# apache/datafusion

Hardware: AMD Instinct MI355X
Metric: tpch_q3_hash_join_rows_per_sec (higher is better)
Workload: dtype int64 keys / decimal128 payload; 1 GPU; INNER hash-join orders⋈lineitem on o_orderkey, TPC-H SF100, Q3 payload (o_orderdate,o_shippriority,l_orderkey,l_extendedprice,l_discount), device-resident inputs; build_rows=150000000, probe_rows=599960064, output_rows=599960064, join_table=rank_map, probe=single_pass_unordered, parallelism=single GPU, exchange=none

## Files before the change

### datafusion_amd/csrc/internal.hpp

```cpp
#pragma once
#include <atomic>
#include <hip/hip_runtime.h>

#include <chrono>
#include <cstdint>
#include <cstring>
#include <map>
#include <memory>
#include <mutex>
#include <stdexcept>
#include <string>
#include <thread>
#include <vector>

#include "../../include/dfgpu.h"

namespace dfgpu {

struct Error : std::runtime_error {
  using std::runtime_error::runtime_error;
};

void set_last_error(const std::string& msg);

// ... 236 lines not shown
  thread_metrics().rows_out += t->nrows;
  return reinterpret_cast<dfgpu_table_t>(t);
}

Column alloc_column(const dfgpu_field& f, const std::string& name, int64_t n, bool with_validity = false);
inline Column alloc_like(const Column& src, int64_t n, bool with_validity = false) {
  Column c = alloc_column(src.field, src.name, n, with_validity);
  c.dict = src.dict;
  return c;
}

inline dfgpu_table_t wrap_quiet(Table* t) { return reinterpret_cast<dfgpu_table_t>(t); }

void scan_mask_popcounts(const uint64_t* mask, const uint64_t* valid, int64_t nrows, uint64_t* out_prefix);
void scan_u32(const uint32_t* in, int64_t n, uint64_t* out_prefix);
void scan_bitmap_words_tab(const uint64_t* words, int64_t n_words, uint64_t* out_prefix, void* out_tab);
uint64_t read_u64(const uint64_t* dev);

Table compact_table(const Table& in, const std::vector<int>& cols, const uint64_t* mask, const uint64_t* mask_valid);
Column gather_column(const Column& in, const int64_t* idx, int64_t n, bool idx_may_be_null);
std::vector<Column> gather_columns(const Table& in, const std::vector<int>& cols, const int64_t* idx, int64_t n, bool idx_may_be_null, const uint32_t* idx32 = nullptr);
struct PackLayout;
bool plan_record_layout(const Table& in, const std::vector<int>& cols, PackLayout& L, int& R, std::vector<int>& order);
Column bool_as_u8(const Column& c, int64_t n);
void and_bitmaps(const uint64_t* a, const uint64_t* b, int64_t nw, uint64_t* out);
void count_nulls(Column& c);

struct Datum {
  Column col;
  std::string str;
  bool scalar = false;
// ... 66 lines not shown
```

### datafusion_amd/csrc/join.hip

```cpp
#include <thread>
#include <functional>
#include <cstdlib>

#include "device.hpp"
#include "internal.hpp"
#include "grouped.hpp"

namespace dfgpu {

Table compact_table(const Table& in, const std::vector<int>& cols, const uint64_t* mask, const uint64_t* mask_valid);
void pack_bytes_to_bitmap(const uint8_t* bytes, int64_t n, uint64_t* words);

enum TableKind : int { KIND_HASH = 0, KIND_ARRAY = 1, KIND_RANK = 2, KIND_RADIX = 3, KIND_FLAT = 4, KIND_FLAT16 = 5,
                       KIND_RETURNED = 6 };
template <int KIND> constexpr bool kind_is_flat() { return KIND == KIND_FLAT || KIND == KIND_FLAT16; }
template <int KIND> constexpr bool kind_is_direct() { return KIND == KIND_ARRAY || KIND == KIND_RANK; }

struct FlatLayout {
  int n;
  uint8_t off[MAX_KEYS];
  uint8_t width[MAX_KEYS];
  int8_t null_bit[MAX_KEYS];
};
constexpr double RANK_MAP_MIN_KEY_DENSITY = 1.0 / 256.0;
// ... 38 lines not shown
  const uint64_t* rank_prefix;
  const uint32_t* rank_perm;
  uint64_t am_offset, am_size, hash_mask;
  int null_equals_null;
  int force_collisions;
  const uint64_t* row_mask;
  const uint4* flat;
  FlatLayout flat_layout;
  int flat_shift;
  uint64_t flat_mask;
  const uint32_t* ret_dest;
  const uint8_t* ret_rec;
  int ret_R;
};

constexpr int ROWPRED_MAX = 2;
struct RowPred {
  const void* data[ROWPRED_MAX];
  const uint64_t* valid[ROWPRED_MAX];
  long long lit[ROWPRED_MAX];
  uint8_t width[ROWPRED_MAX], is_unsigned[ROWPRED_MAX], op[ROWPRED_MAX];
  int n;
};
template <bool NT, int W>
__device__ __forceinline__ void rowpred_load_words(const RowPred& q, int i, int64_t w0, int64_t np, unsigned lane, long long (&v)[W]) {
  const int width = q.width[i];
  if (width == 8) {
    const long long* d = reinterpret_cast<const long long*>(q.data[i]);
#pragma unroll
    for (int j = 0; j < W; j++) {
// ... 184 lines not shown
      lo[j] = load_key<KT>(k, i < n ? i : n - 1);
    }
#pragma unroll
    for (int j = 0; j < BUILD_UNROLL; j++) {
      int64_t i = i0 + j * stride;
      ok[j] = i < n;
      if (HASV) ok[j] = ok[j] && bit_at(k.valid, i < n ? i : n - 1);
    }
#pragma unroll
    for (int j = 0; j < BUILD_UNROLL; j++) {
      if (!ok[j]) continue;
      const uint64_t idx = lo[j] - offset;
      const unsigned long long bit = 1ull << (idx & 63);
      (void)__hip_atomic_fetch_or(&bits[idx >> 6], bit, __ATOMIC_RELAXED, __HIP_MEMORY_SCOPE_AGENT);
    }
  }
}
template <int KT, bool HASV>
__global__ __launch_bounds__(BLOCK) void k_rank_setbytes(KeyCol k, int64_t n, uint64_t offset, uint8_t* __restrict__ bytes) {
  const int64_t stride = (int64_t)gridDim.x * BLOCK;
  for (int64_t i0 = (int64_t)blockIdx.x * BLOCK + threadIdx.x; i0 < n; i0 += stride * BUILD_UNROLL) {
    uint64_t lo[BUILD_UNROLL];
#pragma unroll
    for (int j = 0; j < BUILD_UNROLL; j++) {
      const int64_t i = i0 + j * stride;
      lo[j] = load_key<KT>(k, i < n ? i : n - 1);
    }
#pragma unroll
    for (int j = 0; j < BUILD_UNROLL; j++) {
      const int64_t i = i0 + j * stride;
// ... 20 lines not shown
    const uint64_t idx = gkeys[i] - offset;
    const unsigned long long bit = 1ull << (idx & 63);
    const unsigned long long old = atomicOr(&rb_words[(idx >> 6) - w0], bit);
    dup |= (old & bit) != 0;
  }
  if (dup) *dup_flag = 1;
  __syncthreads();
  for (int i = threadIdx.x; i < nw; i += RB_THREADS) {
    const unsigned long long w = rb_words[i];
    if (i == 0 || i == nw - 1) {
      if (w) atomicOr(&bits[w0 + i], w);
    } else {
      bits[w0 + i] = w;
    }
  }
}
__global__ __launch_bounds__(BLOCK) void k_rank_interleave(const uint64_t* __restrict__ bits, const uint64_t* __restrict__ prefix, int64_t n_words, ulonglong2* __restrict__ tab) {
  for (int64_t w = (int64_t)blockIdx.x * BLOCK + threadIdx.x; w < n_words; w += (int64_t)gridDim.x * BLOCK) tab[w] = make_ulonglong2(bits[w], prefix[w]);
}
__global__ __launch_bounds__(BLOCK) void k_rank_perm_tab(KeyCol k, int64_t n, uint64_t offset, const ulonglong2* __restrict__ tab, uint32_t* __restrict__ perm) {
  for (int64_t i = (int64_t)blockIdx.x * BLOCK + threadIdx.x; i < n; i += (int64_t)gridDim.x * BLOCK) {
    if (k.valid && !bit_at(k.valid, i)) continue;
    uint64_t lo, hi;
    load_words(k, i, lo, hi);
    const uint64_t idx = lo - offset;
    const ulonglong2 e = tab[idx >> 6];
    perm[(uint32_t)e.y + (uint32_t)__popcll(e.x & ((1ull << (idx & 63)) - 1ull))] = (uint32_t)i;
  }
}

// ... 355 lines not shown
    ok[j] = p < np;
    idx[j] = (keys_in ? keys_in[j] : load_key<KT, NT>(k, ok[j] ? p : np - 1)) - c.am_offset;
    if (pre) ok[j] = ok[j] && pre[j];
    else if (c.row_mask) ok[j] = ok[j] && ((c.row_mask[w0 + j] >> lane) & 1ull);
  }
  if (k.valid) {
    uint64_t vw[N];
#pragma unroll
    for (int j = 0; j < N; j++) {
      const int64_t p = ((w0 + j) << 6) + lane;
      vw[j] = k.valid[(p < np ? p : np - 1) >> 6];
    }
#pragma unroll
    for (int j = 0; j < N; j++) ok[j] = ok[j] && ((vw[j] >> lane) & 1ull);
  }
  const uint64_t* tab = c.rank_bits;
  uint64_t bits[N];
#pragma unroll
  for (int j = 0; j < N; j++) {
    ok[j] = ok[j] && idx[j] < c.am_size;
    bits[j] = tab[ok[j] ? (idx[j] >> 6) : 0];
  }
#pragma unroll
  for (int j = 0; j < N; j++) word[j] = ballot64(ok[j] && ((bits[j] >> (idx[j] & 63)) & 1ull));
}

__device__ __forceinline__ uint32_t out_count(int join_type, uint32_t nmatch) {
  switch (join_type) {
    case DFGPU_JOIN_INNER: case DFGPU_JOIN_LEFT: return nmatch;
    case DFGPU_JOIN_RIGHT: case DFGPU_JOIN_FULL: return nmatch ? nmatch : 1u;
    case DFGPU_JOIN_RIGHT_SEMI: return nmatch ? 1u : 0u;
    case DFGPU_JOIN_RIGHT_ANTI: return nmatch ? 0u : 1u;
    case DFGPU_JOIN_RIGHT_MARK: return 1u;
    default: return 0u;
  }
}
// ... 573 lines not shown
  __syncthreads();
  const uint32_t round_rows = agg - base < (uint32_t)EL_CAP ? agg - base : (uint32_t)EL_CAP;
  for (uint32_t q0 = threadIdx.x; q0 < round_rows; q0 += BLOCK) {
    const uint32_t q = base + q0;
    const int64_t prow = (w_base << 6) + s_row[q0];
    int64_t brow = 0;
    uint64_t key = 0;
    if (cols.n_build > 0 || cols.key_col >= 0) {
      key = load_key<KT>(k, prow);
      if (cols.n_build > 0) {
        const uint64_t idx = key - c.am_offset;
        if (KIND == KIND_ARRAY) {
          brow = (int64_t)c.heads[idx] - 1;
        } else {
          uint64_t bw, pre;
          if (c.rank_tab) {
            const ulonglong2 e = c.rank_tab[idx >> 6];
            bw = e.x;
            pre = e.y;
          } else {
            bw = c.rank_bits[idx >> 6];
            pre = c.rank_prefix[idx >> 6];
          }
          const uint32_t rank = (uint32_t)pre + (uint32_t)__popcll(bw & ((1ull << (idx & 63)) - 1ull));
          brow = c.rank_perm ? (int64_t)c.rank_perm[rank] : (int64_t)rank;
        }
      }
    }
    const int64_t d = (int64_t)(out0 + q);
#pragma unroll
    for (int c0 = 0; c0 < MAX_JOIN_COLS; c0 += 4) {
      if (c0 >= cols.n) continue;
      uint4 v[4];
#pragma unroll
      for (int u = 0; u < 4; u++) {
        if (c0 + u >= cols.n) continue;
        int ci = c0 + u + cols.n_build;
        if (ci >= cols.n) ci -= cols.n;
// ... 339 lines not shown
  }
  if (kind == KIND_RETURNED) {
    f(std::integral_constant<int, KIND_RETURNED>{}, std::integral_constant<int, KT_ANY>{});
    return;
  }
  with_key_type(probe_key_type, [&](auto kt) {
    if (kind == KIND_ARRAY) f(std::integral_constant<int, KIND_ARRAY>{}, kt);
    else f(std::integral_constant<int, KIND_RANK>{}, kt);
  });
}

static void ensure_rank_tab(JoinTable& jt) {
  if (jt.kind != KIND_RANK) return;
  std::lock_guard<std::mutex> lk(jt.tab_mu);
  if (jt.rank_tab) return;
  Runtime& r = rt();
  const int64_t n_words = (int64_t)((jt.am_size - 1) >> 6) + 1;
  BufPtr tab = make_buf((size_t)n_words * 16);
  {
    ProfileScope ps("join_build_rank_interleave", n_words * 16);
    k_rank_interleave<<<grid_for(n_words, BLOCK), BLOCK, 0, r.stream>>>(jt.rank_bits->as<uint64_t>(), jt.rank_prefix->as<uint64_t>(), n_words, tab->as<ulonglong2>());
    DFGPU_HIP(hipGetLastError());
  }
  call_epilogue();
  jt.rank_tab = tab;
  std::lock_guard<std::mutex> lk2(jt.mu);
  jt.info.table_bytes += n_words * 16;
}

static void ensure_rank_perm(JoinTable& jt) {
  if (jt.kind != KIND_RANK || !jt.rank_needs_perm) return;
  ensure_rank_tab(jt);
  std::lock_guard<std::mutex> lk(jt.mu);
  if (jt.rank_perm) return;
  Runtime& r = rt();
  const int64_t nb = jt.build.nrows;
  const KeySet ks = make_keyset(jt.build, jt.key_cols);
  BufPtr perm = make_buf((size_t)std::max<int64_t>(nb, 1) * 4);
  {
    ProfileScope ps("join_build_rank_perm", nb * (ks.c[0].width + 4));
    k_rank_perm_tab<<<grid_for(nb, BLOCK), BLOCK, 0, r.stream>>>(ks.c[0], nb, jt.am_offset, jt.rank_tab->as<ulonglong2>(), perm->as<uint32_t>());
    DFGPU_HIP(hipGetLastError());
// ... 4 lines not shown
}

static ProbeCtx make_ctx(JoinTable& jt, const Table& probe, const std::vector<int>& pk, bool need_build_rows = true, bool want_tab = true) {
  if (want_tab) ensure_rank_tab(jt);
  if (need_build_rows) ensure_rank_perm(jt);
  ProbeCtx c{};
  c.bkeys = make_keyset(jt.build, jt.key_cols);
  c.pkeys = make_keyset(probe, pk);
  for (int i = 0; i < c.bkeys.n; i++) {
    int bt = c.bkeys.c[i].type == DFGPU_DATE32 ? DFGPU_INT32 : c.bkeys.c[i].type;
    int pt = c.pkeys.c[i].type == DFGPU_DATE32 ? DFGPU_INT32 : c.pkeys.c[i].type;
    DFGPU_CHECK(bt == pt, "join key types differ between build and probe side (the planner inserts casts)");
  }
  c.heads = jt.heads ? jt.heads->as<uint32_t>() : nullptr;
  c.next = jt.next ? jt.next->as<uint32_t>() : nullptr;
  c.rank_tab = jt.rank_tab ? jt.rank_tab->as<ulonglong2>() : nullptr;
  c.rank_bits = jt.rank_bits ? jt.rank_bits->as<uint64_t>() : nullptr;
  c.rank_prefix = jt.rank_prefix ? jt.rank_prefix->as<uint64_t>() : nullptr;
  c.rank_perm = need_build_rows && jt.rank_perm ? jt.rank_perm->as<uint32_t>() : nullptr;
  c.am_offset = jt.am_offset;
  c.am_size = jt.am_size;
  c.hash_mask = jt.hash_mask;
  c.flat = jt.flat ? jt.flat->as<uint4>() : nullptr;
  c.flat_layout = jt.flat_layout;
  c.flat_shift = jt.flat_shift;
  c.flat_mask = jt.flat_mask;
  c.null_equals_null = jt.null_equality == DFGPU_NULL_EQUALS_NULL;
  c.force_collisions = jt.force_collisions;
  return c;
}

static Column mark_column(const uint8_t* bytes, int64_t n) {
  dfgpu_field f{};
// ... 154 lines not shown
        std::atomic_store(&const_cast<Column&>(kc).stats, std::make_shared<ColStats>(ColStats{res.smin, res.smax, (int64_t)res.valid, res.unsorted == 0, res.descends == 0}));
      }
    }
  }
  const double dense = have_stats ? (double)nb / ((double)range + 1.0) : 0.0;
  bool am_ok = have_stats && !(range >= (uint64_t)opts.perfect_hash_join_small_build_threshold && dense <= opts.perfect_hash_join_min_key_density);
  if (opts.table_mode == 2) am_ok = have_stats;
  am_ok = am_ok && range < (1ull << 34);
  bool rank_ok = have_stats && (opts.table_mode == 0 || opts.table_mode == 3) && range < (1ull << 40) &&
                 (range < (uint64_t)opts.perfect_hash_join_small_build_threshold || dense >= RANK_MAP_MIN_KEY_DENSITY || opts.table_mode == 3);
  DFGPU_CHECK(!speculated || rank_ok, "internal: speculative build statistics outside the rank map's gate");
  DFGPU_CHECK(!(opts.table_mode == 2 && !am_ok), "direct-address join table requested but not applicable");
  DFGPU_CHECK(!(opts.table_mode == 3 && !rank_ok), "rank-map join table requested but not applicable");
  constexpr int64_t MALL_BYTES = (int64_t)256 << 20;

  BufPtr flag = make_zero_buf(4);
  int dup = 0;
  bool flat_wide = false;
  if (rank_ok && !ascending && !speculated && opts.table_mode == 0 && opts.probe_mode == 4 && ks.n == 1 && nb * 8 > MALL_BYTES && nb >= ((int64_t)1 << 22)) {
    const int64_t m = (int64_t)1 << 18;
    const uint64_t slots = (uint64_t)1 << 20;
    BufPtr table = make_zero_buf((size_t)slots * 8);
    {
      ProfileScope ps("join_build_sample_duplicates", m * 2 * ks.c[0].width);
      with_key_type(ks.c[0].type, [&](auto kt) {
        k_sample_duplicates<decltype(kt)::value><<<grid_for(2 * m, BLOCK), BLOCK, 0, r.stream>>>(ks.c[0], nb, nb / m, m, table->as<unsigned long long>(), slots - 1, flag->as<int>());
      });
      DFGPU_HIP(hipGetLastError());
    }
    int seen = 0;
    d2h(&seen, flag->ptr, 4);
    if (seen) {
      dup = 1;
      rank_ok = false;
      DFGPU_HIP(hipMemsetAsync(flag->ptr, 0, 4, r.stream));
    }
  }
  if (rank_ok) {
    const int64_t n_words = (int64_t)(range >> 6) + 1;
    jt->rank_bits = make_zero_buf((size_t)n_words * 8);
    {
      ProfileScope ps("join_build_rank_map", nb * ks.c[0].width);
      int g = std::min(grid_for(nb, BLOCK * BUILD_UNROLL), 2048);
      unsigned long long* bits = jt->rank_bits->as<unsigned long long>();
      KeyCol kc0 = ks.c[0];
      BufPtr grouped_keys;
      constexpr int RB_BITS = 10;
      const bool lds_bits = !ascending && nb > (1 << 22) && n_words * 8 > ((int64_t)16 << 20) && (range >> RB_BITS) < (1ull << 20) - 64;
      if (lds_bits) {
        const GroupSpec gs = group_spec((uint64_t)kmin, range + 1, 1 << RB_BITS);
        GroupedRows gr = group_rows_by_key(kc0, nb, gs, RB_BITS, nullptr, true, false, {}, {}, "join_build_group_keys");
        const int P = 1 << RB_BITS;
        std::vector<uint64_t> gfirst((size_t)P + 1);
        uint64_t max_span = 0;
        for (int q = 0; q <= P; q++) {
          const unsigned __int128 v = ((((unsigned __int128)(unsigned)q) << 64) + gs.mul - 1) / gs.mul;
          gfirst[(size_t)q] = v > (unsigned __int128)(range + 1) || q == P ? range + 1 : (uint64_t)v;
          if (q) max_span = std::max(max_span, gfirst[(size_t)q] - gfirst[(size_t)q - 1]);
        }
        BufPtr d_first = make_buf(gfirst.size() * 8);
        h2d_async(d_first->ptr, gfirst.data(), gfirst.size() * 8);
        const size_t lds = (size_t)((max_span >> 6) + 2) * 8;
        DFGPU_HIP(hipFuncSetAttribute(reinterpret_cast<const void*>(k_rank_bits_grouped), hipFuncAttributeMaxDynamicSharedMemorySize, (int)lds));
        k_rank_bits_grouped<<<P, RB_THREADS, lds, r.stream>>>(gr.keys->as<uint64_t>(), gr.bounds->as<uint64_t>(), d_first->as<uint64_t>(), (uint64_t)kmin, bits, flag->as<int>());
        DFGPU_HIP(hipGetLastError());
        DFGPU_HIP(hipStreamSynchronize(r.stream));
      } else {
      if (!ascending && !kc0.valid && kc0.width == 8 && nb > (1 << 22) && n_words * 8 > ((int64_t)16 << 20)) {
        const Column& kcol = build.cols[(size_t)key_cols[0]];
        grouped_keys = kcol.data;
        if (kcol.data_offset != 0) {
          grouped_keys = make_buf((size_t)nb * 8);
          DFGPU_HIP(hipMemcpyAsync(grouped_keys->ptr, kcol.ptr(), (size_t)nb * 8, hipMemcpyDeviceToDevice, r.stream));
        }
        int range_bits = 0;
        while (range_bits < 64 && ((range + 1) >> range_bits)) range_bits++;
        radix_group_keys(grouped_keys, nb, std::max(0, range_bits - 6), 6);
        kc0.data = grouped_keys->ptr;
      }
      const bool byte_map = !ascending && nb > (1 << 20) && range < (1ull << 32);
      if (byte_map) {
        BufPtr bytes = make_zero_buf((size_t)n_words * 64);
        with_key_type(kc0.type, [&](auto kt) {
          constexpr int T = decltype(kt)::value;
          if (kc0.valid) k_rank_setbytes<T, true><<<g, BLOCK, 0, r.stream>>>(kc0, nb, (uint64_t)kmin, bytes->as<uint8_t>());
          else k_rank_setbytes<T, false><<<g, BLOCK, 0, r.stream>>>(kc0, nb, (uint64_t)kmin, bytes->as<uint8_t>());
        });
        DFGPU_HIP(hipGetLastError());
        pack_bytes_to_bitmap(bytes->as<uint8_t>(), n_words * 64, jt->rank_bits->as<uint64_t>());
      } else {
      with_key_type(kc0.type, [&](auto kt) {
        constexpr int T = decltype(kt)::value;
        if (speculated) k_rank_setbits<T, false, true, true><<<g, BLOCK, 0, r.stream>>>(kc0, nb, (uint64_t)kmin, bits, flag->as<int>(), range);
        else if (ascending) k_rank_setbits<T, false, true><<<g, BLOCK, 0, r.stream>>>(kc0, nb, (uint64_t)kmin, bits, flag->as<int>());
        else if (kc0.valid) k_rank_setbits<T, true, false><<<g, BLOCK, 0, r.stream>>>(kc0, nb, (uint64_t)kmin, bits, flag->as<int>());
        else k_rank_setbits<T, false, false><<<g, BLOCK, 0, r.stream>>>(kc0, nb, (uint64_t)kmin, bits, flag->as<int>());
      });
      }
      }
    }
    jt->rank_prefix = make_buf((size_t)(n_words + 1) * 8);
    BufPtr eager_tab;
    if (ascending && (double)nb >= 0.15 * ((double)range + 1.0) && option_on("join.eager_rank_tab", true)) {
      eager_tab = make_buf((size_t)n_words * 16);
      scan_bitmap_words_tab(jt->rank_bits->as<uint64_t>(), n_words, jt->rank_prefix->as<uint64_t>(), eager_tab->ptr);
    } else
    scan_mask_popcounts(jt->rank_bits->as<uint64_t>(), nullptr, n_words * 64, jt->rank_prefix->as<uint64_t>());
    if (!ascending) dup = (int64_t)read_u64(jt->rank_prefix->as<uint64_t>() + n_words) != n_valid_keys;
    if (speculated) {
      int wrong = 0;
      d2h(&wrong, flag->ptr, 4);
      if (wrong) {
        ProfileScope ps("join_build_speculation_missed", 0);
        jt.reset();
        return join_build_fixed_keys(build, key_cols, null_equality, opts, false);
      }
      std::atomic_store(&const_cast<Column&>(build.cols[key_cols[0]]).stats,
                        std::make_shared<ColStats>(ColStats{kmin, (long long)((uint64_t)kmin + range), nb, true, true}));
    }
    if (!dup) {
      jt->kind = KIND_RANK;
      jt->am_offset = (uint64_t)kmin;
      jt->am_size = range + 1;
      jt->rank_needs_perm = !ascending;
      jt->info.table_bytes = n_words * 16;
      if (eager_tab) {
        jt->rank_tab = eager_tab;
        jt->info.table_bytes += n_words * 16;
      }
    } else {
      DFGPU_CHECK(opts.table_mode != 3, "rank-map join table requested but the build keys are not unique");
      jt->rank_bits.reset();
      jt->rank_prefix.reset();
    }
  }
  if (opts.table_mode == 0 && dup && opts.probe_mode == 4 && ks.n == 1 && nb * 8 > MALL_BYTES) {
    jt->rank_bits.reset();
    jt->kind = KIND_RADIX;
    jt->radix = radix_join_build(build, key_cols, null_equality == DFGPU_NULL_EQUALS_NULL, jt->force_collisions);
    jt->keys_unique = false;
    jt->info.table_bytes = radix_join_table_bytes(*jt->radix);
    jt->info.table_kind = KIND_RADIX;
    jt->info.build_keys_unique = 0;
    return jt;
  }
  if (jt->kind != KIND_RANK && am_ok) {
    jt->kind = KIND_ARRAY;
    jt->array_map = true;
    jt->am_offset = (uint64_t)kmin;
    jt->am_size = range + 1;
    jt->heads = make_zero_buf(jt->am_size * 4);
    auto am_build = [&](uint32_t* next) {
      const int g = std::min(grid_for(nb, BLOCK * BUILD_UNROLL), 2048);
      with_key_type(ks.c[0].type, [&](auto kt) {
        constexpr int T = decltype(kt)::value;
        if (ks.c[0].valid) k_am_build<T, true><<<g, BLOCK, 0, r.stream>>>(ks.c[0], nb, jt->am_offset, jt->heads->as<uint32_t>(), next, flag->as<int>());
        else k_am_build<T, false><<<g, BLOCK, 0, r.stream>>>(ks.c[0], nb, jt->am_offset, jt->heads->as<uint32_t>(), next, flag->as<int>());
      });
    };
    if (dup) jt->next = make_zero_buf((size_t)nb * 4);
    {
      ProfileScope ps("join_build_array_map", nb * ks.c[0].width);
      am_build(dup ? jt->next->as<uint32_t>() : nullptr);
    }
    if (!dup) {
      d2h(&dup, flag->ptr, 4);
      if (dup && opts.table_mode == 0 && opts.probe_mode == 4 && ks.n == 1 && nb * 8 > MALL_BYTES) {
        jt->heads.reset();
        jt->array_map = false;
        jt->kind = KIND_RADIX;
        jt->radix = radix_join_build(build, key_cols, null_equality == DFGPU_NULL_EQUALS_NULL, jt->force_collisions);
        jt->keys_unique = false;
        jt->info.table_bytes = radix_join_table_bytes(*jt->radix);
        jt->info.table_kind = KIND_RADIX;
        jt->info.build_keys_unique = 0;
        return jt;
      }
      if (dup) {
        DFGPU_HIP(hipMemsetAsync(jt->heads->ptr, 0, jt->am_size * 4, r.stream));
        jt->next = make_zero_buf((size_t)nb * 4);
        ProfileScope ps("join_build_array_map", nb * ks.c[0].width);
// ... 11 lines not shown
      log2cap++;
    }
    jt->flat_mask = cap - 1;
    jt->flat_shift = 64 - log2cap;
    jt->next = make_zero_buf((size_t)(nb ? nb : 1) * 4);
    jt->flat = make_buf((size_t)cap * (flat_wide ? 32 : 16));
    BufPtr owner = make_zero_buf((size_t)cap * 4);
    BufPtr more = make_zero_buf((size_t)(nb ? nb : 1) * 4);
    int64_t kb = 0;
    for (int i = 0; i < ks.n; i++) kb += nb * ks.c[i].width;
    const int nen = null_equality == DFGPU_NULL_EQUALS_NULL;
    {
      ProfileScope ps("join_build_flat_table", kb + nb * 4 + (int64_t)cap * (flat_wide ? 32 : 16));
      if (nb) {
        const int g = grid_for(nb, BLOCK);
        if (flat_wide) k_flat_claim<true><<<g, BLOCK, 0, r.stream>>>(ks, jt->flat_layout, nb, nen, jt->force_collisions, jt->flat_shift, jt->flat_mask, owner->as<uint32_t>(), jt->next->as<uint32_t>(), flag->as<int>(), more->as<uint32_t>());
        else k_flat_claim<false><<<g, BLOCK, 0, r.stream>>>(ks, jt->flat_layout, nb, nen, jt->force_collisions, jt->flat_shift, jt->flat_mask, owner->as<uint32_t>(), jt->next->as<uint32_t>(), flag->as<int>(), more->as<uint32_t>());
      }
      const int gf = grid_for((int64_t)cap, BLOCK);
      if (flat_wide) k_flat_fill<true><<<gf, BLOCK, 0, r.stream>>>(ks, jt->flat_layout, (int64_t)cap, nen, owner->as<uint32_t>(), more->as<uint32_t>(), jt->flat->as<uint4>());
      else k_flat_fill<false><<<gf, BLOCK, 0, r.stream>>>(ks, jt->flat_layout, (int64_t)cap, nen, owner->as<uint32_t>(), more->as<uint32_t>(), jt->flat->as<uint4>());
      DFGPU_HIP(hipGetLastError());
    }
    d2h(&dup, flag->ptr, 4);
    jt->info.table_bytes = (int64_t)cap * (flat_wide ? 32 : 16) + nb * 4;
  } else if (jt->kind != KIND_RANK) {
    DFGPU_CHECK(opts.table_mode != 5, "flat (inline-key) join table requested but the key columns do not pack into 16 bytes");
    jt->kind = KIND_HASH;
    dup = 0;
    uint64_t cap = 64;
    while (cap < (uint64_t)nb * 2) cap <<= 1;
    jt->hash_mask = cap - 1;
    jt->heads = make_zero_buf(cap * 4);
    jt->next = make_zero_buf((size_t)(nb ? nb : 1) * 4);
    if (nb) {
      int64_t kb = 0;
      for (int i = 0; i < ks.n; i++) kb += nb * ks.c[i].width;
      {
        ProfileScope ps("join_build_hash_map", kb + nb * 8);
        k_hm_build<<<grid_for(nb, BLOCK), BLOCK, 0, r.stream>>>(ks, nb, jt->hash_mask, null_equality == DFGPU_NULL_EQUALS_NULL, jt->force_collisions,
                                                                jt->heads->as<uint32_t>(), jt->next->as<uint32_t>());
      }
      ProfileScope ps("join_build_check_unique", kb + nb * 4);
      k_hm_check_unique<<<grid_for(nb, BLOCK), BLOCK, 0, r.stream>>>(ks, nb, null_equality == DFGPU_NULL_EQUALS_NULL, jt->next->as<uint32_t>(), flag->as<int>());
      d2h(&dup, flag->ptr, 4);
    }
    jt->info.table_bytes = (int64_t)cap * 4 + nb * 4;
  }
  DFGPU_HIP(hipGetLastError());
  jt->keys_unique = dup == 0;
  jt->info.used_array_map = jt->kind == KIND_ARRAY;
  jt->info.build_keys_unique = jt->keys_unique;
  jt->info.table_kind = jt->kind;
  jt->info.build_keys_ascending = ascending;
  return jt;
}

static Table with_build_dictionaries(const JoinTable& jt, const Table& probe, std::vector<int>& pk) {
  DFGPU_CHECK(pk.size() == jt.key_cols.size(), "probe key count differs from build key count");
  Table fixed;
// ... 314 lines not shown
        jt.info.probe_rows += probe.nrows;
        jt.info.output_rows += fused.nrows;
        return fused;
      }
    }
    return join_probe_with_filter(jt, probe, pk, join_type, bout, pout, nullptr);
  }
  const int64_t np = probe.nrows;
  const int64_t n_words = (np + 63) / 64;
  int kind = jt.kind;
  ProbeCtx ctx = make_ctx(jt, probe, pk, false, false);
  auto need_tab = [&]() {
    if (jt.kind == KIND_RANK) {
      ensure_rank_tab(jt);
      ctx.rank_tab = jt.rank_tab->as<ulonglong2>();
    }
  };
  for (int c : bout) DFGPU_CHECK(c >= 0 && c < (int)jt.build.cols.size(), "build output column out of range");
  for (int c : pout) DFGPU_CHECK(c >= 0 && c < (int)probe.cols.size(), "probe output column out of range");
  uint8_t* visited = nullptr;
  if (needs_visited(join_type)) {
    {
      std::lock_guard<std::mutex> lk(jt.mu);
      if (!jt.visited) {
        jt.visited = make_zero_buf((size_t)jt.build.nrows + 64);
        DFGPU_HIP(hipStreamSynchronize(rt().stream));
      }
    }
    visited = jt.visited->as<uint8_t>();
  }
// ... 242 lines not shown
      }
      if (r.profiling) {
        std::lock_guard<std::mutex> lk(r.mu);
        r.recs.push_back(Runtime::Rec{want_single ? "join_probe_fused" : "join_probe_placed", ea, eb, bytes, std::this_thread::get_id()});
        r.recs.push_back(Runtime::Rec{"join_probe_shared_columns", sa, sb, 0, std::this_thread::get_id()});
      }
      out.nrows = np;
      jt.info.output_rows += out.nrows;
      return out;
    }
    speculate = speculate && fused_mode == FUSED_PLACED && !listed;
    if (fused_mode == FUSED_PLACED && !speculate) {
      BufPtr counts = make_buf((size_t)n_tiles * 4);
      state = make_buf((size_t)(n_tiles + 1) * 8);
      if (listed) out_words = make_buf((size_t)n_words * 8);
      {
        ProfileScope ps("join_probe_tile_counts", key_bytes + (pred_in_counts ? np * lazy->pred_bytes_per_row : 0));
        with_kind_and_key(kind, ctx.pkeys.c[0].type, [&](auto kd, auto kt) {
          constexpr int K = decltype(kd)::value, T = decltype(kt)::value;
          if constexpr (kind_is_direct<K>()) {
            const bool nt = option_on("join.counts_nt", true);
            if (pred_in_counts) {
              if (nt) k_join_tile_counts<K, T, FUSED_W, true, true><<<(unsigned)n_tiles, BLOCK, 0, r.stream>>>(ctx, np, invert, nullptr, counts->as<uint32_t>(), out_words->as<uint64_t>(), lazy->pred);
              else k_join_tile_counts<K, T, FUSED_W, true><<<(unsigned)n_tiles, BLOCK, 0, r.stream>>>(ctx, np, invert, nullptr, counts->as<uint32_t>(), out_words->as<uint64_t>(), lazy->pred);
              return;
            }
            if (nt) {
              k_join_tile_counts<K, T, FUSED_W, false, true><<<(unsigned)n_tiles, BLOCK, 0, r.stream>>>(ctx, np, invert, row_mask, counts->as<uint32_t>(), out_words ? out_words->as<uint64_t>() : nullptr);
              return;
            }
// ... 918 lines not shown
```

### datafusion_amd/csrc/scan.hip

```cpp
#include "device.hpp"
#include "internal.hpp"

namespace dfgpu {

constexpr int SCAN_ITEMS = 8;
constexpr int SCAN_CHUNK = BLOCK * SCAN_ITEMS;

struct InU32 {
  const uint32_t* p;
  __device__ __forceinline__ uint32_t operator()(int64_t i) const { return p[i]; }
};
struct InMaskPopc {
  const uint64_t* mask;
  const uint64_t* valid;
  int64_t nrows;
  __device__ __forceinline__ uint32_t operator()(int64_t w) const {
    uint64_t m = mask[w];
    if (valid) m &= valid[w];
    int64_t rem = nrows - w * 64;
    if (rem < 64) m &= (rem <= 0) ? 0ull : ((~0ull) >> (64 - rem));
    return (uint32_t)__popcll(m);
  }
};

// ... 82 lines not shown
    const uint64_t excl = lookback_exclusive(state, tile, tot);
    if (threadIdx.x == 0) {
      s_excl = excl;
      if (tile == n_tiles - 1) out[n] = excl + tot;
    }
  }
  __syncthreads();
  ex += s_excl;
#pragma unroll
  for (int j = 0; j < CH_ITEMS; j++) {
    if (base + j < n) out[base + j] = ex;
    ex += v[j];
  }
}

__global__ __launch_bounds__(BLOCK) void k_scan_down_tab(InMaskPopc in, int64_t n, const uint64_t* chunk_base, uint64_t* out, ulonglong2* __restrict__ tab) {
  int64_t base = (int64_t)blockIdx.x * SCAN_CHUNK + (int64_t)threadIdx.x * SCAN_ITEMS;
  uint64_t w[SCAN_ITEMS];
  uint64_t s = 0;
#pragma unroll
  for (int j = 0; j < SCAN_ITEMS; j++) {
    w[j] = base + j < n ? in.mask[base + j] : 0ull;
    s += (uint32_t)__popcll(w[j]);
  }
  uint64_t tot;
  uint64_t ex = block_exclusive_scan(s, &tot) + chunk_base[blockIdx.x];
#pragma unroll
  for (int j = 0; j < SCAN_ITEMS; j++) {
    if (base + j < n) {
      out[base + j] = ex;
      tab[base + j] = make_ulonglong2(w[j], ex);
    }
    ex += (uint32_t)__popcll(w[j]);
  }
}

template <typename In>
static void run_scan(In in, int64_t n, uint64_t* out, const char* name) {
  Runtime& r = rt();
  if (n == 0) {
    DFGPU_HIP(hipMemsetAsync(out, 0, 8, r.stream));
    return;
  }
  const int64_t n_tiles_ch = (n + CH_CHUNK - 1) / CH_CHUNK;
  if (n_tiles_ch <= option_int("scan.chained_max_tiles", 8)) {
    const int64_t n_tiles = n_tiles_ch;
    BufPtr state = make_zero_buf((size_t)(n_tiles + 2) * 8);
    ProfileScope ps(name, 0);
    k_scan_chained<<<(unsigned)n_tiles, BLOCK, 0, r.stream>>>(in, n, state->as<uint64_t>(), reinterpret_cast<unsigned*>(state->as<uint64_t>() + n_tiles), out);
    DFGPU_HIP(hipGetLastError());
    return;
  }
  int64_t n_chunks = (n + SCAN_CHUNK - 1) / SCAN_CHUNK;
  BufPtr sums = make_buf((size_t)n_chunks * 8);
  ProfileScope ps(name, 0);
  k_scan_reduce<<<(unsigned)n_chunks, BLOCK, 0, r.stream>>>(in, n, sums->as<uint64_t>());
  k_scan_sums<<<1, BLOCK, 0, r.stream>>>(sums->as<uint64_t>(), n_chunks, out + n);
  k_scan_down<<<(unsigned)n_chunks, BLOCK, 0, r.stream>>>(in, n, sums->as<uint64_t>(), out);
  DFGPU_HIP(hipGetLastError());
}

void scan_mask_popcounts(const uint64_t* mask, const uint64_t* valid, int64_t nrows, uint64_t* out_prefix) {
  int64_t n_words = (nrows + 63) / 64;
  run_scan(InMaskPopc{mask, valid, nrows}, n_words, out_prefix, "scan_mask_popcounts");
}
void scan_u32(const uint32_t* in, int64_t n, uint64_t* out_prefix) { run_scan(InU32{in}, n, out_prefix, "scan_u32"); }
void scan_bitmap_words_tab(const uint64_t* words, int64_t n_words, uint64_t* out_prefix, void* out_tab) {
  Runtime& r = rt();
  DFGPU_CHECK(n_words > 0, "scan_bitmap_words_tab: empty bitmap");
  const InMaskPopc in{words, nullptr, n_words * 64};
  const int64_t n_chunks = (n_words + SCAN_CHUNK - 1) / SCAN_CHUNK;
  BufPtr sums = make_buf((size_t)n_chunks * 8);
  ProfileScope ps("scan_mask_popcounts", 0);
  k_scan_reduce<<<(unsigned)n_chunks, BLOCK, 0, r.stream>>>(in, n_words, sums->as<uint64_t>());
  k_scan_sums<<<1, BLOCK, 0, r.stream>>>(sums->as<uint64_t>(), n_chunks, out_prefix + n_words);
  k_scan_down_tab<<<(unsigned)n_chunks, BLOCK, 0, r.stream>>>(in, n_words, sums->as<uint64_t>(), out_prefix, reinterpret_cast<ulonglong2*>(out_tab));
  DFGPU_HIP(hipGetLastError());
}

}
```

Measured before the change: 311.3 billion rows/s.

## Build rank-map table in one pass from sorted build keys

```diff
diff --git a/datafusion_amd/csrc/internal.hpp b/datafusion_amd/csrc/internal.hpp
--- a/datafusion_amd/csrc/internal.hpp
+++ b/datafusion_amd/csrc/internal.hpp
@@ -274,7 +274,6 @@
 
 void scan_mask_popcounts(const uint64_t* mask, const uint64_t* valid, int64_t nrows, uint64_t* out_prefix);
 void scan_u32(const uint32_t* in, int64_t n, uint64_t* out_prefix);
-void scan_bitmap_words_tab(const uint64_t* words, int64_t n_words, uint64_t* out_prefix, void* out_tab);
 uint64_t read_u64(const uint64_t* dev);
 
 Table compact_table(const Table& in, const std::vector<int>& cols, const uint64_t* mask, const uint64_t* mask_valid);
diff --git a/datafusion_amd/csrc/join.hip b/datafusion_amd/csrc/join.hip
--- a/datafusion_amd/csrc/join.hip
+++ b/datafusion_amd/csrc/join.hip
@@ -76,6 +76,18 @@
   int ret_R;
 };
 
+__device__ __forceinline__ uint64_t rank_word(const ProbeCtx& c, uint64_t w) { return c.rank_bits ? c.rank_bits[w] : c.rank_tab[w].x; }
+__device__ __forceinline__ void rank_entry(const ProbeCtx& c, uint64_t w, uint64_t& bits, uint64_t& prefix) {
+  if (c.rank_tab) {
+    const ulonglong2 e = c.rank_tab[w];
+    bits = e.x;
+    prefix = e.y;
+  } else {
+    bits = c.rank_bits[w];
+    prefix = c.rank_prefix[w];
+  }
+}
+
 constexpr int ROWPRED_MAX = 2;
 struct RowPred {
   const void* data[ROWPRED_MAX];
@@ -290,6 +302,122 @@
       const unsigned long long bit = 1ull << (idx & 63);
       (void)__hip_atomic_fetch_or(&bits[idx >> 6], bit, __ATOMIC_RELAXED, __HIP_MEMORY_SCOPE_AGENT);
     }
+  }
+}
+typedef unsigned long long rt_u64x2 __attribute__((ext_vector_type(2)));
+typedef unsigned rt_u32x4 __attribute__((ext_vector_type(4)));
+template <int KT>
+__device__ __forceinline__ void load_keys4(const KeyCol& k, int64_t i0, uint64_t (&out)[4]) {
+  if (KT == KT_I64 && ((uintptr_t)k.data & 15) == 0) {
+    const rt_u64x2* p = reinterpret_cast<const rt_u64x2*>((const uint64_t*)k.data + i0);
+    const rt_u64x2 a = __builtin_nontemporal_load(p), b = __builtin_nontemporal_load(p + 1);
+    out[0] = a.x; out[1] = a.y; out[2] = b.x; out[3] = b.y;
+  } else if ((KT == KT_I32 || KT == KT_U32) && ((uintptr_t)k.data & 15) == 0) {
+    const rt_u32x4 a = __builtin_nontemporal_load(reinterpret_cast<const rt_u32x4*>((const uint32_t*)k.data + i0));
+    out[0] = KT == KT_I32 ? (uint64_t)(int64_t)(int32_t)a.x : a.x;
+    out[1] = KT == KT_I32 ? (uint64_t)(int64_t)(int32_t)a.y : a.y;
+    out[2] = KT == KT_I32 ? (uint64_t)(int64_t)(int32_t)a.z : a.z;
+    out[3] = KT == KT_I32 ? (uint64_t)(int64_t)(int32_t)a.w : a.w;
+  } else {
+#pragma unroll
+    for (int j = 0; j < 4; j++) out[j] = load_key<KT, true>(k, i0 + j);
+  }
+}
+constexpr int RT_ROWS = 4096;
+constexpr int RT_WIN = 1024;
+constexpr int RT_LANE_ROWS = 4;
+constexpr int RT_CHUNK = WAVE * RT_LANE_ROWS;
+constexpr int RT_STEPS = RT_ROWS / RT_CHUNK / (BLOCK / WAVE);
+template <int KT, bool VERIFY>
+__global__ __launch_bounds__(BLOCK) void k_rank_tab_onepass(KeyCol k, int64_t n, uint64_t offset, uint64_t range, ulonglong2* __restrict__ tab, int* __restrict__ flag) {
+  __shared__ unsigned long long s_bits[RT_WIN];
+  __shared__ unsigned s_first[RT_WIN];
+  constexpr int WAVES = BLOCK / WAVE;
+  const unsigned lane = lane_id();
+  const int wv = threadIdx.x >> 6;
+  const int64_t r0 = (int64_t)blockIdx.x * RT_ROWS;
+  const int64_t r1 = r0 + RT_ROWS < n ? r0 + RT_ROWS : n;
+  const uint64_t n_words = (range >> 6) + 1;
+  uint64_t idx[RT_STEPS][RT_LANE_ROWS], pidx[RT_STEPS];
+#pragma unroll
+  for (int c = 0; c < RT_STEPS; c++) {
+    const int64_t i0 = r0 + (int64_t)(c * WAVES + wv) * RT_CHUNK + lane * RT_LANE_ROWS;
+    if (i0 + RT_LANE_ROWS <= n) {
+      load_keys4<KT>(k, i0, idx[c]);
+#pragma unroll
+      for (int j = 0; j < RT_LANE_ROWS; j++) idx[c][j] -= offset;
+    } else {
+#pragma unroll
+      for (int j = 0; j < RT_LANE_ROWS; j++) idx[c][j] = load_key<KT, true>(k, i0 + j < n ? i0 + j : n - 1) - offset;
+    }
+    pidx[c] = 0;
+    if (VERIFY) pidx[c] = load_key<KT>(k, i0 < n ? (i0 > 0 ? i0 - 1 : 0) : n - 1) - offset;
+  }
+  const bool tail_lane = wv == WAVES - 1 && r1 + lane < n;
+  const uint64_t tail_idx = tail_lane ? load_key<KT>(k, r1 + lane) - offset : ~0ull;
+  const uint64_t w_first = r0 > 0 ? ((load_key<KT>(k, r0 - 1) - offset) >> 6) + 1 : 0ull;
+  const uint64_t w_last = (load_key<KT>(k, r1 - 1) - offset) >> 6;
+  const uint64_t w_end = w_last < n_words ? w_last : n_words - 1;
+  const int cnt = w_end < w_first ? 0 : (w_end - w_first + 1 < (uint64_t)RT_WIN ? (int)(w_end - w_first + 1) : RT_WIN);
+  for (int t = threadIdx.x; t < cnt; t += BLOCK) {
+    s_bits[t] = 0ull;
+    s_first[t] = ~0u;
+  }
+  __syncthreads();
+  auto put = [&](uint64_t w, unsigned long long bits, int64_t row, bool first_known, bool is_first) {
+    const uint64_t slot = w - w_first;
+    if (slot < (uint64_t)cnt) {
+      atomicOr(&s_bits[slot], bits);
+      atomicMin(&s_first[slot], (unsigned)(row - r0));
+    } else {
+      unsigned long long* e = reinterpret_cast<unsigned long long*>(tab + w);
+      (void)__hip_atomic_fetch_or(e, bits, __ATOMIC_RELAXED, __HIP_MEMORY_SCOPE_AGENT);
+      if (!first_known) is_first = row == 0 || ((load_key<KT>(k, row - 1) - offset) >> 6) != w;
+      if (is_first) e[1] = (unsigned long long)row;
+    }
+  };
+#pragma unroll
+  for (int c = 0; c < RT_STEPS; c++) {
+    const int64_t i0 = r0 + (int64_t)(c * WAVES + wv) * RT_CHUNK + lane * RT_LANE_ROWS;
+    bool ok[RT_LANE_ROWS], later[RT_LANE_ROWS];
+    uint64_t w = ~0ull, v = 0ull;
+    unsigned rel = 0;
+    bool found = false, bad = false, any_later = false;
+#pragma unroll
+    for (int j = 0; j < RT_LANE_ROWS; j++) {
+      const uint64_t x = idx[c][j];
+      if (VERIFY) bad = bad || (i0 + j < r1 && (x > range || (i0 + j > 0 && x <= (j ? idx[c][j - 1] : pidx[c]))));
+      ok[j] = i0 + j < r1 && x <= range && (x >> 6) >= w_first;
+      if (ok[j] && !found) {
+        found = true;
+        w = x >> 6;
+        rel = (unsigned)(i0 + j - r0);
+      }
+      const bool lead = ok[j] && (x >> 6) == w;
+      v |= lead ? 1ull << (x & 63) : 0ull;
+      later[j] = ok[j] && !lead;
+      any_later = any_later || later[j];
+    }
+    if (VERIFY && ballot64(bad) != 0 && lane == 0) atomicOr(flag, 1);
+    const uint64_t inc = wave_inclusive_sum_dpp(v);
+    const uint64_t w_next = __shfl_down(w, 1, 64);
+    const uint64_t tails = ballot64(lane == 63 || w_next != w);
+    const uint64_t heads = (tails << 1) | 1ull;
+    const int head_lane = 63 - __builtin_clzll(heads & ((2ull << lane) - 1ull));
+    const uint64_t before = __shfl(inc - v, head_lane, 64);
+    const unsigned head_rel = __shfl(rel, head_lane, 64);
+    if (found && ((tails >> lane) & 1ull)) put(w, inc - before, r0 + head_rel, false, false);
+    if (any_later) {
+#pragma unroll
+      for (int j = 1; j < RT_LANE_ROWS; j++)
+        if (later[j]) put(idx[c][j] >> 6, 1ull << (idx[c][j] & 63), i0 + j, true, (idx[c][j - 1] >> 6) != (idx[c][j] >> 6));
+    }
+  }
+  if (tail_lane && tail_idx <= range && (tail_idx >> 6) == w_last && w_last >= w_first) put(w_last, 1ull << (tail_idx & 63), r1 + lane, true, false);
+  __syncthreads();
+  for (int t = threadIdx.x; t < cnt; t += BLOCK) {
+    const unsigned long long b = s_bits[t];
+    tab[w_first + t] = make_ulonglong2(b, b ? (unsigned long long)(r0 + s_first[t]) : 0ull);
   }
 }
 template <int KT, bool HASV>
@@ -340,6 +468,9 @@
       bits[w0 + i] = w;
     }
   }
+}
+__global__ __launch_bounds__(BLOCK) void k_rank_deinterleave(const ulonglong2* __restrict__ tab, int64_t n_words, uint64_t* __restrict__ bits) {
+  for (int64_t w = (int64_t)blockIdx.x * BLOCK + threadIdx.x; w < n_words; w += (int64_t)gridDim.x * BLOCK) bits[w] = tab[w].x;
 }
 __global__ __launch_bounds__(BLOCK) void k_rank_interleave(const uint64_t* __restrict__ bits, const uint64_t* __restrict__ prefix, int64_t n_words, ulonglong2* __restrict__ tab) {
   for (int64_t w = (int64_t)blockIdx.x * BLOCK + threadIdx.x; w < n_words; w += (int64_t)gridDim.x * BLOCK) tab[w] = make_ulonglong2(bits[w], prefix[w]);
@@ -725,12 +856,11 @@
 #pragma unroll
     for (int j = 0; j < N; j++) ok[j] = ok[j] && ((vw[j] >> lane) & 1ull);
   }
-  const uint64_t* tab = c.rank_bits;
   uint64_t bits[N];
 #pragma unroll
   for (int j = 0; j < N; j++) {
     ok[j] = ok[j] && idx[j] < c.am_size;
-    bits[j] = tab[ok[j] ? (idx[j] >> 6) : 0];
+    bits[j] = rank_word(c, ok[j] ? (idx[j] >> 6) : 0);
   }
 #pragma unroll
   for (int j = 0; j < N; j++) word[j] = ballot64(ok[j] && ((bits[j] >> (idx[j] & 63)) & 1ull));
@@ -1334,14 +1464,7 @@
           brow = (int64_t)c.heads[idx] - 1;
         } else {
           uint64_t bw, pre;
-          if (c.rank_tab) {
-            const ulonglong2 e = c.rank_tab[idx >> 6];
-            bw = e.x;
-            pre = e.y;
-          } else {
-            bw = c.rank_bits[idx >> 6];
-            pre = c.rank_prefix[idx >> 6];
-          }
+          rank_entry(c, idx >> 6, bw, pre);
           const uint32_t rank = (uint32_t)pre + (uint32_t)__popcll(bw & ((1ull << (idx & 63)) - 1ull));
           brow = c.rank_perm ? (int64_t)c.rank_perm[rank] : (int64_t)rank;
         }
@@ -1711,6 +1834,7 @@
   if (jt.kind != KIND_RANK) return;
   std::lock_guard<std::mutex> lk(jt.tab_mu);
   if (jt.rank_tab) return;
+  DFGPU_CHECK(jt.rank_bits && jt.rank_prefix, "internal: rank map without a table and without bitmap + prefix");
   Runtime& r = rt();
   const int64_t n_words = (int64_t)((jt.am_size - 1) >> 6) + 1;
   BufPtr tab = make_buf((size_t)n_words * 16);
@@ -1723,6 +1847,25 @@
   jt.rank_tab = tab;
   std::lock_guard<std::mutex> lk2(jt.mu);
   jt.info.table_bytes += n_words * 16;
+}
+
+static void ensure_rank_bits(JoinTable& jt) {
+  if (jt.kind != KIND_RANK) return;
+  std::lock_guard<std::mutex> lk(jt.tab_mu);
+  if (jt.rank_bits) return;
+  DFGPU_CHECK(jt.rank_tab != nullptr, "internal: rank map without a table and without bitmap + prefix");
+  Runtime& r = rt();
+  const int64_t n_words = (int64_t)((jt.am_size - 1) >> 6) + 1;
+  BufPtr bits = make_buf((size_t)n_words * 8);
+  {
+    ProfileScope ps("join_build_rank_deinterleave", n_words * 24);
+    k_rank_deinterleave<<<grid_for(n_words, BLOCK), BLOCK, 0, r.stream>>>(jt.rank_tab->as<ulonglong2>(), n_words, bits->as<uint64_t>());
+    DFGPU_HIP(hipGetLastError());
+  }
+  call_epilogue();
+  jt.rank_bits = bits;
+  std::lock_guard<std::mutex> lk2(jt.mu);
+  jt.info.table_bytes += n_words * 8;
 }
 
 static void ensure_rank_perm(JoinTable& jt) {
@@ -1757,9 +1900,13 @@
   }
   c.heads = jt.heads ? jt.heads->as<uint32_t>() : nullptr;
   c.next = jt.next ? jt.next->as<uint32_t>() : nullptr;
-  c.rank_tab = jt.rank_tab ? jt.rank_tab->as<ulonglong2>() : nullptr;
-  c.rank_bits = jt.rank_bits ? jt.rank_bits->as<uint64_t>() : nullptr;
-  c.rank_prefix = jt.rank_prefix ? jt.rank_prefix->as<uint64_t>() : nullptr;
+  {
+    std::lock_guard<std::mutex> lk(jt.tab_mu);
+    c.rank_tab = jt.rank_tab ? jt.rank_tab->as<ulonglong2>() : nullptr;
+    c.rank_bits = jt.rank_bits ? jt.rank_bits->as<uint64_t>() : nullptr;
+    c.rank_prefix = jt.rank_prefix ? jt.rank_prefix->as<uint64_t>() : nullptr;
+    DFGPU_CHECK(jt.kind != KIND_RANK || c.rank_tab || (c.rank_bits && c.rank_prefix), "internal: rank map without a table and without bitmap + prefix");
+  }
   c.rank_perm = need_build_rows && jt.rank_perm ? jt.rank_perm->as<uint32_t>() : nullptr;
   c.am_offset = jt.am_offset;
   c.am_size = jt.am_size;
@@ -1944,7 +2091,11 @@
   DFGPU_CHECK(!(opts.table_mode == 3 && !rank_ok), "rank-map join table requested but not applicable");
   constexpr int64_t MALL_BYTES = (int64_t)256 << 20;
 
-  BufPtr flag = make_zero_buf(4);
+  BufPtr flag;
+  auto need_flag = [&]() {
+    if (!flag) flag = make_zero_buf(4);
+    return flag->as<int>();
+  };
   int dup = 0;
   bool flat_wide = false;
   if (rank_ok && !ascending && !speculated && opts.table_mode == 0 && opts.probe_mode == 4 && ks.n == 1 && nb * 8 > MALL_BYTES && nb >= ((int64_t)1 << 22)) {
@@ -1954,20 +2105,32 @@
     {
       ProfileScope ps("join_build_sample_duplicates", m * 2 * ks.c[0].width);
       with_key_type(ks.c[0].type, [&](auto kt) {
-        k_sample_duplicates<decltype(kt)::value><<<grid_for(2 * m, BLOCK), BLOCK, 0, r.stream>>>(ks.c[0], nb, nb / m, m, table->as<unsigned long long>(), slots - 1, flag->as<int>());
+        k_sample_duplicates<decltype(kt)::value><<<grid_for(2 * m, BLOCK), BLOCK, 0, r.stream>>>(ks.c[0], nb, nb / m, m, table->as<unsigned long long>(), slots - 1, need_flag());
       });
       DFGPU_HIP(hipGetLastError());
     }
     int seen = 0;
-    d2h(&seen, flag->ptr, 4);
+    d2h(&seen, need_flag(), 4);
     if (seen) {
       dup = 1;
       rank_ok = false;
-      DFGPU_HIP(hipMemsetAsync(flag->ptr, 0, 4, r.stream));
+      DFGPU_HIP(hipMemsetAsync(need_flag(), 0, 4, r.stream));
     }
   }
   if (rank_ok) {
     const int64_t n_words = (int64_t)(range >> 6) + 1;
+    BufPtr eager_tab;
+    if (ascending && (double)nb >= 0.15 * ((double)range + 1.0)) {
+      eager_tab = make_zero_buf((size_t)n_words * 16);
+      ProfileScope ps("join_build_rank_tab_onepass", nb * ks.c[0].width + n_words * 16);
+      const int g = (int)((nb + RT_ROWS - 1) / RT_ROWS);
+      with_key_type(ks.c[0].type, [&](auto kt) {
+        constexpr int T = decltype(kt)::value;
+        if (speculated) k_rank_tab_onepass<T, true><<<g, BLOCK, 0, r.stream>>>(ks.c[0], nb, (uint64_t)kmin, range, eager_tab->as<ulonglong2>(), need_flag());
+        else k_rank_tab_onepass<T, false><<<g, BLOCK, 0, r.stream>>>(ks.c[0], nb, (uint64_t)kmin, range, eager_tab->as<ulonglong2>(), nullptr);
+      });
+      DFGPU_HIP(hipGetLastError());
+    } else {
     jt->rank_bits = make_zero_buf((size_t)n_words * 8);
     {
       ProfileScope ps("join_build_rank_map", nb * ks.c[0].width);
@@ -1992,7 +2155,7 @@
         h2d_async(d_first->ptr, gfirst.data(), gfirst.size() * 8);
         const size_t lds = (size_t)((max_span >> 6) + 2) * 8;
         DFGPU_HIP(hipFuncSetAttribute(reinterpret_cast<const void*>(k_rank_bits_grouped), hipFuncAttributeMaxDynamicSharedMemorySize, (int)lds));
-        k_rank_bits_grouped<<<P, RB_THREADS, lds, r.stream>>>(gr.keys->as<uint64_t>(), gr.bounds->as<uint64_t>(), d_first->as<uint64_t>(), (uint64_t)kmin, bits, flag->as<int>());
+        k_rank_bits_grouped<<<P, RB_THREADS, lds, r.stream>>>(gr.keys->as<uint64_t>(), gr.bounds->as<uint64_t>(), d_first->as<uint64_t>(), (uint64_t)kmin, bits, need_flag());
         DFGPU_HIP(hipGetLastError());
         DFGPU_HIP(hipStreamSynchronize(r.stream));
       } else {
@@ -2021,25 +2184,21 @@
       } else {
       with_key_type(kc0.type, [&](auto kt) {
         constexpr int T = decltype(kt)::value;
-        if (speculated) k_rank_setbits<T, false, true, true><<<g, BLOCK, 0, r.stream>>>(kc0, nb, (uint64_t)kmin, bits, flag->as<int>(), range);
-        else if (ascending) k_rank_setbits<T, false, true><<<g, BLOCK, 0, r.stream>>>(kc0, nb, (uint64_t)kmin, bits, flag->as<int>());
-        else if (kc0.valid) k_rank_setbits<T, true, false><<<g, BLOCK, 0, r.stream>>>(kc0, nb, (uint64_t)kmin, bits, flag->as<int>());
-        else k_rank_setbits<T, false, false><<<g, BLOCK, 0, r.stream>>>(kc0, nb, (uint64_t)kmin, bits, flag->as<int>());
+        if (speculated) k_rank_setbits<T, false, true, true><<<g, BLOCK, 0, r.stream>>>(kc0, nb, (uint64_t)kmin, bits, need_flag(), range);
+        else if (ascending) k_rank_setbits<T, false, true><<<g, BLOCK, 0, r.stream>>>(kc0, nb, (uint64_t)kmin, bits, need_flag());
+        else if (kc0.valid) k_rank_setbits<T, true, false><<<g, BLOCK, 0, r.stream>>>(kc0, nb, (uint64_t)kmin, bits, need_flag());
+        else k_rank_setbits<T, false, false><<<g, BLOCK, 0, r.stream>>>(kc0, nb, (uint64_t)kmin, bits, need_flag());
       });
       }
       }
     }
     jt->rank_prefix = make_buf((size_t)(n_words + 1) * 8);
-    BufPtr eager_tab;
-    if (ascending && (double)nb >= 0.15 * ((double)range + 1.0) && option_on("join.eager_rank_tab", true)) {
-      eager_tab = make_buf((size_t)n_words * 16);
-      scan_bitmap_words_tab(jt->rank_bits->as<uint64_t>(), n_words, jt->rank_prefix->as<uint64_t>(), eager_tab->ptr);
-    } else
     scan_mask_popcounts(jt->rank_bits->as<uint64_t>(), nullptr, n_words * 64, jt->rank_prefix->as<uint64_t>());
     if (!ascending) dup = (int64_t)read_u64(jt->rank_prefix->as<uint64_t>() + n_words) != n_valid_keys;
+    }
     if (speculated) {
       int wrong = 0;
-      d2h(&wrong, flag->ptr, 4);
+      d2h(&wrong, need_flag(), 4);
       if (wrong) {
         ProfileScope ps("join_build_speculation_missed", 0);
         jt.reset();
@@ -2054,10 +2213,7 @@
       jt->am_size = range + 1;
       jt->rank_needs_perm = !ascending;
       jt->info.table_bytes = n_words * 16;
-      if (eager_tab) {
-        jt->rank_tab = eager_tab;
-        jt->info.table_bytes += n_words * 16;
-      }
+      jt->rank_tab = eager_tab;
     } else {
       DFGPU_CHECK(opts.table_mode != 3, "rank-map join table requested but the build keys are not unique");
       jt->rank_bits.reset();
@@ -2084,8 +2240,8 @@
       const int g = std::min(grid_for(nb, BLOCK * BUILD_UNROLL), 2048);
       with_key_type(ks.c[0].type, [&](auto kt) {
         constexpr int T = decltype(kt)::value;
-        if (ks.c[0].valid) k_am_build<T, true><<<g, BLOCK, 0, r.stream>>>(ks.c[0], nb, jt->am_offset, jt->heads->as<uint32_t>(), next, flag->as<int>());
-        else k_am_build<T, false><<<g, BLOCK, 0, r.stream>>>(ks.c[0], nb, jt->am_offset, jt->heads->as<uint32_t>(), next, flag->as<int>());
+        if (ks.c[0].valid) k_am_build<T, true><<<g, BLOCK, 0, r.stream>>>(ks.c[0], nb, jt->am_offset, jt->heads->as<uint32_t>(), next, need_flag());
+        else k_am_build<T, false><<<g, BLOCK, 0, r.stream>>>(ks.c[0], nb, jt->am_offset, jt->heads->as<uint32_t>(), next, need_flag());
       });
     };
     if (dup) jt->next = make_zero_buf((size_t)nb * 4);
@@ -2094,7 +2250,7 @@
       am_build(dup ? jt->next->as<uint32_t>() : nullptr);
     }
     if (!dup) {
-      d2h(&dup, flag->ptr, 4);
+      d2h(&dup, need_flag(), 4);
       if (dup && opts.table_mode == 0 && opts.probe_mode == 4 && ks.n == 1 && nb * 8 > MALL_BYTES) {
         jt->heads.reset();
         jt->array_map = false;
@@ -2136,15 +2292,15 @@
       ProfileScope ps("join_build_flat_table", kb + nb * 4 + (int64_t)cap * (flat_wide ? 32 : 16));
       if (nb) {
         const int g = grid_for(nb, BLOCK);
-        if (flat_wide) k_flat_claim<true><<<g, BLOCK, 0, r.stream>>>(ks, jt->flat_layout, nb, nen, jt->force_collisions, jt->flat_shift, jt->flat_mask, owner->as<uint32_t>(), jt->next->as<uint32_t>(), flag->as<int>(), more->as<uint32_t>());
-        else k_flat_claim<false><<<g, BLOCK, 0, r.stream>>>(ks, jt->flat_layout, nb, nen, jt->force_collisions, jt->flat_shift, jt->flat_mask, owner->as<uint32_t>(), jt->next->as<uint32_t>(), flag->as<int>(), more->as<uint32_t>());
+        if (flat_wide) k_flat_claim<true><<<g, BLOCK, 0, r.stream>>>(ks, jt->flat_layout, nb, nen, jt->force_collisions, jt->flat_shift, jt->flat_mask, owner->as<uint32_t>(), jt->next->as<uint32_t>(), need_flag(), more->as<uint32_t>());
+        else k_flat_claim<false><<<g, BLOCK, 0, r.stream>>>(ks, jt->flat_layout, nb, nen, jt->force_collisions, jt->flat_shift, jt->flat_mask, owner->as<uint32_t>(), jt->next->as<uint32_t>(), need_flag(), more->as<uint32_t>());
       }
       const int gf = grid_for((int64_t)cap, BLOCK);
       if (flat_wide) k_flat_fill<true><<<gf, BLOCK, 0, r.stream>>>(ks, jt->flat_layout, (int64_t)cap, nen, owner->as<uint32_t>(), more->as<uint32_t>(), jt->flat->as<uint4>());
       else k_flat_fill<false><<<gf, BLOCK, 0, r.stream>>>(ks, jt->flat_layout, (int64_t)cap, nen, owner->as<uint32_t>(), more->as<uint32_t>(), jt->flat->as<uint4>());
       DFGPU_HIP(hipGetLastError());
     }
-    d2h(&dup, flag->ptr, 4);
+    d2h(&dup, need_flag(), 4);
     jt->info.table_bytes = (int64_t)cap * (flat_wide ? 32 : 16) + nb * 4;
   } else if (jt->kind != KIND_RANK) {
     DFGPU_CHECK(opts.table_mode != 5, "flat (inline-key) join table requested but the key columns do not pack into 16 bytes");
@@ -2164,8 +2320,8 @@
                                                                 jt->heads->as<uint32_t>(), jt->next->as<uint32_t>());
       }
       ProfileScope ps("join_build_check_unique", kb + nb * 4);
-      k_hm_check_unique<<<grid_for(nb, BLOCK), BLOCK, 0, r.stream>>>(ks, nb, null_equality == DFGPU_NULL_EQUALS_NULL, jt->next->as<uint32_t>(), flag->as<int>());
-      d2h(&dup, flag->ptr, 4);
+      k_hm_check_unique<<<grid_for(nb, BLOCK), BLOCK, 0, r.stream>>>(ks, nb, null_equality == DFGPU_NULL_EQUALS_NULL, jt->next->as<uint32_t>(), need_flag());
+      d2h(&dup, need_flag(), 4);
     }
     jt->info.table_bytes = (int64_t)cap * 4 + nb * 4;
   }
@@ -2510,6 +2666,12 @@
     if (jt.kind == KIND_RANK) {
       ensure_rank_tab(jt);
       ctx.rank_tab = jt.rank_tab->as<ulonglong2>();
+    }
+  };
+  auto need_bits = [&]() {
+    if (jt.kind == KIND_RANK) {
+      ensure_rank_bits(jt);
+      ctx.rank_bits = jt.rank_bits->as<uint64_t>();
     }
   };
   for (int c : bout) DFGPU_CHECK(c >= 0 && c < (int)jt.build.cols.size(), "build output column out of range");
@@ -2782,6 +2944,7 @@
       BufPtr counts = make_buf((size_t)n_tiles * 4);
       state = make_buf((size_t)(n_tiles + 1) * 8);
       if (listed) out_words = make_buf((size_t)n_words * 8);
+      if (kind == KIND_RANK) need_bits();
       {
         ProfileScope ps("join_probe_tile_counts", key_bytes + (pred_in_counts ? np * lazy->pred_bytes_per_row : 0));
         with_kind_and_key(kind, ctx.pkeys.c[0].type, [&](auto kd, auto kt) {
diff --git a/datafusion_amd/csrc/scan.hip b/datafusion_amd/csrc/scan.hip
--- a/datafusion_amd/csrc/scan.hip
+++ b/datafusion_amd/csrc/scan.hip
@@ -120,27 +120,6 @@
   }
 }
 
-__global__ __launch_bounds__(BLOCK) void k_scan_down_tab(InMaskPopc in, int64_t n, const uint64_t* chunk_base, uint64_t* out, ulonglong2* __restrict__ tab) {
-  int64_t base = (int64_t)blockIdx.x * SCAN_CHUNK + (int64_t)threadIdx.x * SCAN_ITEMS;
-  uint64_t w[SCAN_ITEMS];
-  uint64_t s = 0;
-#pragma unroll
-  for (int j = 0; j < SCAN_ITEMS; j++) {
-    w[j] = base + j < n ? in.mask[base + j] : 0ull;
-    s += (uint32_t)__popcll(w[j]);
-  }
-  uint64_t tot;
-  uint64_t ex = block_exclusive_scan(s, &tot) + chunk_base[blockIdx.x];
-#pragma unroll
-  for (int j = 0; j < SCAN_ITEMS; j++) {
-    if (base + j < n) {
-      out[base + j] = ex;
-      tab[base + j] = make_ulonglong2(w[j], ex);
-    }
-    ex += (uint32_t)__popcll(w[j]);
-  }
-}
-
 template <typename In>
 static void run_scan(In in, int64_t n, uint64_t* out, const char* name) {
   Runtime& r = rt();
@@ -171,17 +150,5 @@
   run_scan(InMaskPopc{mask, valid, nrows}, n_words, out_prefix, "scan_mask_popcounts");
 }
 void scan_u32(const uint32_t* in, int64_t n, uint64_t* out_prefix) { run_scan(InU32{in}, n, out_prefix, "scan_u32"); }
-void scan_bitmap_words_tab(const uint64_t* words, int64_t n_words, uint64_t* out_prefix, void* out_tab) {
-  Runtime& r = rt();
-  DFGPU_CHECK(n_words > 0, "scan_bitmap_words_tab: empty bitmap");
-  const InMaskPopc in{words, nullptr, n_words * 64};
-  const int64_t n_chunks = (n_words + SCAN_CHUNK - 1) / SCAN_CHUNK;
-  BufPtr sums = make_buf((size_t)n_chunks * 8);
-  ProfileScope ps("scan_mask_popcounts", 0);
-  k_scan_reduce<<<(unsigned)n_chunks, BLOCK, 0, r.stream>>>(in, n_words, sums->as<uint64_t>());
-  k_scan_sums<<<1, BLOCK, 0, r.stream>>>(sums->as<uint64_t>(), n_chunks, out_prefix + n_words);
-  k_scan_down_tab<<<(unsigned)n_chunks, BLOCK, 0, r.stream>>>(in, n_words, sums->as<uint64_t>(), out_prefix, reinterpret_cast<ulonglong2*>(out_tab));
-  DFGPU_HIP(hipGetLastError());
-}
 
 }
```

Measured after the change: 337.9 billion rows/s, median of 6. 8.5% higher.
